# Vill-Lab/2023-TIFS-ISTVT

Measured on AMD Instinct MI355X. Metric: clips/sec (BxTx3x224x224 fwd+bwd), higher is better.
Workload: dtype bf16; 1 GPU; C2: B=32/GPU T=8 224x224 full ISTVT (Xception stem + 12-layer DSTTr) train step (fwd+bwd+grad all-reduce+SGD), random-init weights; global_batch=32, frames=8, size=224, depth=12, parallelism=dp1, early_allreduce=False, attn_fp8=False, dead_row_elimination=False, final_norm_class_rows_only=False, optimizer=SGD(momentum 0.9) fused, step_graphs=False

## Files before the change

2023-tifs-istvt_amd/_lib.py:

```python
import ctypes
import os
from ctypes import c_float, c_int, c_long, c_void_p

_HERE = os.path.dirname(os.path.abspath(__file__))
LIB_PATH = os.environ.get('ISTVT_LIB') or os.path.join(_HERE, 'libistvt_hip.so')

P, I, L, F = c_void_p, c_int, c_long, c_float

SIGNATURES = {
    'istvt_gemm': [P, L, I, P, L, I, P, L, I, I, I, P, P, L, P, I, I, I, F, P, P, I, I, P],
    'istvt_layernorm_fwd': [P, L, P, P, P, L, P, P, L, I, F, I, P],
    'istvt_layernorm_fwd_diff': [P, L, P, P, P, L, P, L, P, P, I, I, I, I, F, I, P],
    'istvt_layernorm_bwd': [P, L, P, L, P, P, P, P, L, P, L, P, P, P, P, L, L, I, I, P],
    'istvt_layernorm_bwd_ws_elems': [L, I],
    'istvt_layernorm_bwd_partial': [P, L, P, L, P, P, P, P, L, P, L, I, P, L, L, I, I, P],
    'istvt_layernorm_bwd_reduce': [P, L, L, I, P, P, P, P],
    'istvt_attn_spatial_fwd': [P, L, P, L, P, I, I, I, I, F, I, P],
    'istvt_attn_spatial_bwd': [P, L, P, P, L, P, P, P, I, I, I, I, F, I, P],
    'istvt_attn_spatial_fwd_fp8': [P, L, P, L, P, I, I, I, I, F, I, P],
    'istvt_attn_spatial_bwd_fp8': [P, L, P, P, L, P, P, P, I, I, I, I, F, I, P],
    'istvt_attn_temporal_fwd': [P, L, P, L, P, L, I, I, I, I, I, F, I, I, P],
    'istvt_attn_temporal_bwd': [P, L, P, L, P, L, P, P, I, I, I, I, I, F, I, I, P],
    'istvt_attn_spatial_relevance': [P, L, P, L, P, P, P, I, I, I, I, F, I, P],
    'istvt_attn_temporal_relevance': [P, L, P, L, P, P, I, I, I, I, I, F, I, I, P],
# ... 17 lines not shown
    'istvt_bn_add_fwd': [P, P, P, P, P, L, I, I, P],
    'istvt_im2col_conv1': [P, P, I, I, I, P],
    'istvt_conv1_fwd': [P, P, P, I, I, I, P],
    'istvt_conv1_fwd_u8': [P, P, P, P, P, I, I, I, P],
    'istvt_conv1_wgrad': [P, P, P, P, I, I, I, P],
    'istvt_conv1_wgrad_slabs': [],
    'istvt_conv1_fwd_u8_view': [P, L, I, I, P, P, P, P, P, I, I, I, P],
    'istvt_conv1_wgrad_u8': [P, P, L, I, I, P, P, P, P, P, I, I, I, P],
    'istvt_im2col_conv1_u8': [P, L, I, I, P, P, P, P, I, I, I, P],
    'istvt_crop_resize_u8': [P, L, I, I, P, P, I, I, P],
    'istvt_jpeg_roundtrip_u8': [P, L, I, I, I, P, I, P, L, P, P],
    'istvt_conv2_fwd': [P, P, P, P, I, I, I, P],
    'istvt_conv2_dgrad': [P, P, P, P, P, I, I, I, P],
    'istvt_conv2_wgrad': [P, P, P, P, P, I, I, I, P],
    'istvt_conv2_wgrad_slabs': [],
    'istvt_col2im_conv1': [P, P, I, I, I, P],
    'istvt_im2col3x3': [P, P, I, P, I, I, I, I, I, P],
    'istvt_col2im3x3': [P, P, P, P, I, I, I, I, I, P],
    'istvt_dwconv3x3': [P, P, P, I, I, I, I, P, I, I, P, P, I, I, P, I, I, P, P, I, P],
    'istvt_dwconv3x3_wgrad': [P, P, I, P, P, P, L, I, I, I, I, I, P],
    'istvt_dwconv3x3_wgrad_ws_elems': [I, I, I, I],
    'istvt_pool_add_fwd': [P, P, P, P, P, P, I, I, I, I, I, P],
    'istvt_pool_bwd': [P, P, P, I, I, I, I, P, P, P, P, I, P],
    'istvt_subsample2': [P, P, I, I, I, I, I, P],
    'istvt_splitk_reduce': [P, I, L, P, P],
    'istvt_wgrad_group': [I, P, P, P, P, P, P, P, I, I, P, L, P],
    'istvt_wgrad_group_splits': [I, P, P, I],
    'istvt_colsum': [P, P, L, I, L, P, L, I, P],
    'istvt_colsum_ws_elems': [L, I],
    'istvt_rows_reduce': [P, I, L, P, P],
# ... 63 lines not shown
```

2023-tifs-istvt_amd/csrc/conv_dense.hip:

```cpp
#include "common.h"
#include "u8_view.h"
#include <type_traits>

namespace {

__device__ __forceinline__ bf16x8 ld_frag(const bf16_t* p) { return *reinterpret_cast<const bf16x8*>(p); }
__device__ __forceinline__ bf16x8 zero_frag() {
    bf16x8 f;
#pragma unroll
    for (int i = 0; i < 8; ++i) f[i] = (bf16_t)0.0f;
    return f;
}
__device__ __forceinline__ f32x4 mma16(const bf16x8& a, const bf16x8& b, const f32x4& c) {
    return __builtin_amdgcn_mfma_f32_16x16x32_bf16(a, b, c, 0, 0, 0);
}

template <typename T>
__device__ __forceinline__ void conv1_mac_store(const float* v, const float* __restrict__ w, T* __restrict__ out) {
#pragma unroll
    for (int c8 = 0; c8 < 4; ++c8) {
        float o[8];
#pragma unroll
        for (int j = 0; j < 8; ++j) {
            const float* wc = w + (c8 * 8 + j) * 27;
            float a = 0.f;
#pragma unroll
            for (int k = 0; k < 27; ++k) a = fmaf(wc[k], v[k], a);
            o[j] = a;
        }
        store8(out + c8 * 8, o);
    }
}

template <typename T>
__global__ __launch_bounds__(256) void conv1_fwd_kernel(const float* __restrict__ x, const float* __restrict__ w,
                                                        T* __restrict__ u1, long Mo, int S, int Ho, int Wo) {
    const long m = (long)blockIdx.x * 256 + threadIdx.x;
    if (m >= Mo) return;
    const int xo = (int)(m % Wo), yo = (int)((m / Wo) % Ho);
    const long f = m / ((long)Wo * Ho);
    float v[27];
#pragma unroll
    for (int ci = 0; ci < 3; ++ci)
#pragma unroll
        for (int dy = 0; dy < 3; ++dy) {
            const float* row = x + ((f * 3 + ci) * S + 2 * yo + dy) * S + 2 * xo;
#pragma unroll
            for (int dx = 0; dx < 3; ++dx) v[ci * 9 + dy * 3 + dx] = row[dx];
        }
    conv1_mac_store(v, w, u1 + m * 32);
}

struct Conv1Mac {
    static __device__ __forceinline__ int slot(int dy, int dx, int ci) { return ci * 9 + dy * 3 + dx; }
    template <typename T>
    static __device__ __forceinline__ void emit(const float* v, const float* __restrict__ w, T* __restrict__ out) {
        int w0 = 0;
        asm volatile("" : "+s"(w0));
        conv1_mac_store(v, w + w0, out);
    }
};

struct Conv1Col {
    static __device__ __forceinline__ int slot(int dy, int dx, int ci) { return (dy * 3 + dx) * 3 + ci; }
    template <typename T>
// ... 34 lines not shown
#pragma unroll
        for (int dy = 0; dy < 3; ++dy) {
            const int rr = 2 * yl + dy;
            const unsigned char* row = sb + rr * pitch + u8_row_lead(lead0, rr, rstride);
#pragma unroll
            for (int dx = 0; dx < 3; ++dx) {
                const unsigned char* px = row + u8_view_px(2 * xo + dx, S, vw.flip);
#pragma unroll
                for (int ci = 0; ci < 3; ++ci) v[Sink::slot(dy, dx, ci)] = lut[ci * 256 + px[ci]];
            }
        }
        Sink::emit(v, w, out + ((f * Ho + yb) * (long)Ho + o) * 32);
    }
}

__global__ __launch_bounds__(256, 2) void conv2_fwd_kernel(const bf16_t* __restrict__ u1, const float* __restrict__ bnp,
                                                           const bf16_t* __restrict__ w, bf16_t* __restrict__ u2, long Mo,
                                                           int H, int W, int Ho, int Wo, int ngroups) {
    const int tid = threadIdx.x, lane = tid & 63, wave = tid >> 6;
    const int r = lane & 15, g = lane >> 4;
    __shared__ bf16x8 wl3[9 * 64];
    bf16x8 wf[9][3];
#pragma unroll
    for (int tap = 0; tap < 9; ++tap) {
#pragma unroll
        for (int nt = 0; nt < 3; ++nt)
            wf[tap][nt] = ld_frag(w + (16 * (r >> 2) + 4 * nt + (r & 3)) * 288 + tap * 32 + 8 * g);
        if (wave == 0) wl3[tap * 64 + lane] = ld_frag(w + (16 * (r >> 2) + 4 * 3 + (r & 3)) * 288 + tap * 32 + 8 * g);
    }
    __syncthreads();
    float mu[8], sc[8], be[8];
    load8(bnp + 8 * g, mu);
    load8(bnp + 2 * 32 + 8 * g, sc);
    load8(bnp + 3 * 32 + 8 * g, be);
    constexpr int RSEG = 9;
    const int nstrips = (Wo + 15) / 16, nsegs = (Ho + RSEG - 1) / RSEG;
// ... 37 lines not shown
                        const bf16x8& xf = ring[(k + dy) % 3][dx];
#pragma unroll
                        for (int nt = 0; nt < 3; ++nt) acc[nt] = mma16(wf[dy * 3 + dx][nt], xf, acc[nt]);
                        acc[3] = mma16(wl3[(dy * 3 + dx) * 64 + lo], xf, acc[3]);
                    }
                if (ok) {
                    bf16x8 o0, o1;
#pragma unroll
                    for (int i = 0; i < 4; ++i) {
                        o0[i] = (bf16_t)acc[0][i]; o0[4 + i] = (bf16_t)acc[1][i];
                        o1[i] = (bf16_t)acc[2][i]; o1[4 + i] = (bf16_t)acc[3][i];
                    }
                    bf16_t* dst = u2 + (((f * Ho + yo) * Wo) + xo) * 64 + 16 * g;
                    *reinterpret_cast<bf16x8*>(dst) = o0;
                    *reinterpret_cast<bf16x8*>(dst + 8) = o1;
                }
            }
        }
    }
}

__global__ __launch_bounds__(256, 2) void conv2_dgrad_kernel(const bf16_t* __restrict__ du2, const bf16_t* __restrict__ w,
                                                             const bf16_t* __restrict__ u1, const float* __restrict__ bnp,
                                                             bf16_t* __restrict__ dz1, long Mi, int H, int W, int Ho,
                                                             int Wo, int ngroups) {
    __shared__ bf16_t wt[9 * 32 * 64];
    const int tid = threadIdx.x, lane = tid & 63, wave = tid >> 6;
    const int r = lane & 15, g = lane >> 4;
    for (int i = tid; i < 64 * 36; i += 256) {
        const int co = i / 36, k8 = (i % 36) * 8;
        const bf16x8 v = ld_frag(w + co * 288 + k8);
#pragma unroll
        for (int j = 0; j < 8; ++j) wt[(k8 + j) * 64 + co] = v[j];
    }
    __syncthreads();
    bf16x8 wf[9][2][2];
#pragma unroll
    for (int tap = 3; tap < 9; ++tap)
#pragma unroll
        for (int ks = 0; ks < 2; ++ks)
#pragma unroll
            for (int nt = 0; nt < 2; ++nt)
                wf[tap][ks][nt] = ld_frag(wt + (tap * 32 + 8 * (r >> 2) + 4 * nt + (r & 3)) * 64 + 32 * ks + 8 * g);
// ... 49 lines not shown
#pragma unroll
                    for (int nt = 0; nt < 2; ++nt)
                        acc[nt] = mma16(ld_frag(wt + (dx * 32 + wo + 4 * nt) * 64 + 32 * ks + wcol), ring[k % 3][dx][ks], acc[nt]);
            if (ok) {
                float mu[8], sc[8], be[8];
                load8(bnp + 8 * g, mu);
                load8(bnp + 2 * 32 + 8 * g, sc);
                load8(bnp + 3 * 32 + 8 * g, be);
                bf16x8 o;
#pragma unroll
                for (int j = 0; j < 8; ++j) {
                    const float z = ((float)uraw[j] - mu[j]) * sc[j] + be[j];
                    o[j] = (bf16_t)(z > 0.f ? acc[j >> 2][j & 3] : 0.f);
                }
                *reinterpret_cast<bf16x8*>(dz1 + m * 32 + 8 * g) = o;
            }
            }
        }
    }
}

constexpr int WG_PX = 32;
constexpr int DIMG_PITCH = 64 * 2 + 16;
constexpr int AIMG_PITCH = 32 * 2 + 16;
constexpr int AIMG_ROWS = WG_PX + 2;

__device__ __forceinline__ bf16x8 tr_frag(const char* img, int pitch, int k0, int col16, int r) {
    typedef short4v __attribute__((address_space(3))) * lds_ptr;
    typedef short short8v __attribute__((ext_vector_type(8)));
    const int q = r >> 2, pp = r & 3;
    const char* pa = img + (k0 + q) * pitch + (col16 + 4 * pp) * 2;
    const char* pb = pa + 4 * pitch;
// ... 239 lines not shown
    const int cap = 256 * per_cu;
    return need < cap ? (need > 0 ? need : 1) : cap;
}

}

extern "C" int istvt_conv1_fwd(const float* x, const float* w, void* u1, int Fr, int S, int dtype, hipStream_t stream) {
    if (Fr <= 0 || S < 3) return ISTVT_ERR_SHAPE;
    const int Ho = (S - 3) / 2 + 1;
    const long Mo = (long)Fr * Ho * Ho;
    DISPATCH_DTYPE(dtype, hipLaunchKernelGGL((conv1_fwd_kernel<T>), dim3((unsigned)((Mo + 255) / 256)), dim3(256), 0,
                                             stream, x, w, (T*)u1, Mo, S, Ho, Ho));
    return istvt_check_launch();
}

static inline bool u8_view_args_ok(const void* x, long total, int Hs, int Ws, const float* mean, const float* stdv, int Fr,
                                   int S) {
    if (Fr <= 0 || S < 3 || !x || !mean || !stdv) return false;
    if (Hs < S || Ws < S || Hs > 16384 || Ws > 16384) return false;
    return total >= (long)Fr * Hs * Ws * 3;
}

template <typename Sink>
static int conv1_u8_launch(const void* x, long total, int Hs, int Ws, const int* view, const float* mean, const float* stdv,
                           const float* w, void* out, int Fr, int S, int dtype, hipStream_t stream) {
    if (!u8_view_args_ok(x, total, Hs, Ws, mean, stdv, Fr, S) || S > 4096 || !out) return ISTVT_ERR_SHAPE;
    const int Ho = (S - 3) / 2 + 1;
    const int pitch = u8_row_pitch(S);
    int R = 1;
    double best = 0.0;
// ... 16 lines not shown
                                       hipStream_t stream) {
    if (!w) return ISTVT_ERR_SHAPE;
    return conv1_u8_launch<Conv1Mac>(x, total, Hs, Ws, view, mean, stdv, w, u1, Fr, S, dtype, stream);
}

extern "C" int istvt_conv1_fwd_u8(const void* x, const float* mean, const float* stdv, const float* w, void* u1, int Fr,
                                  int S, int dtype, hipStream_t stream) {
    return istvt_conv1_fwd_u8_view(x, (long)Fr * S * S * 3, S, S, nullptr, mean, stdv, w, u1, Fr, S, dtype, stream);
}

extern "C" int istvt_im2col_conv1_u8(const void* x, long total, int Hs, int Ws, const int* view, const float* mean,
                                     const float* stdv, void* col, int Fr, int S, int dtype, hipStream_t stream) {
    return conv1_u8_launch<Conv1Col>(x, total, Hs, Ws, view, mean, stdv, nullptr, col, Fr, S, dtype, stream);
}

extern "C" int istvt_conv2_fwd(const void* u1, const float* bnp, const void* w, void* u2, int Fr, int H, int W,
                               hipStream_t stream) {
    if (Fr <= 0 || H < 3 || W < 3 || !bnp) return ISTVT_ERR_SHAPE;
    const int Ho = H - 2, Wo = W - 2;
    const long Mo = (long)Fr * Ho * Wo;
    if (Mo / 16 + 1 > 0x7fffffffL) return ISTVT_ERR_SHAPE;
    const int ngroups = (int)((Mo + 15) / 16);
    const long items = (long)Fr * ((Wo + 15) / 16) * ((Ho + 8) / 9);
    hipLaunchKernelGGL(conv2_fwd_kernel, dim3(wave_grid((int)(items < 0x7fffffffL ? items : 0x7fffffffL), 2)), dim3(256), 0, stream, (const bf16_t*)u1, bnp,
                       (const bf16_t*)w, (bf16_t*)u2, Mo, H, W, Ho, Wo, ngroups);
    return istvt_check_launch();
}

extern "C" int istvt_conv2_dgrad(const void* du2, const void* w, const void* u1, const float* bnp, void* dz1, int Fr,
                                 int H, int W, hipStream_t stream) {
    if (Fr <= 0 || H < 3 || W < 3 || !bnp) return ISTVT_ERR_SHAPE;
    const long Mi = (long)Fr * H * W;
    if (Mi / 16 + 1 > 0x7fffffffL) return ISTVT_ERR_SHAPE;
    const int ngroups = (int)((Mi + 15) / 16);
    const long items = (long)Fr * ((W + 15) / 16) * ((H + 8) / 9);
    hipLaunchKernelGGL(conv2_dgrad_kernel, dim3(wave_grid((int)(items < 0x7fffffffL ? items : 0x7fffffffL), 2)), dim3(256), 0, stream, (const bf16_t*)du2,
                       (const bf16_t*)w, (const bf16_t*)u1, bnp, (bf16_t*)dz1, Mi, H, W, H - 2, W - 2, ngroups);
    return istvt_check_launch();
}

extern "C" int istvt_conv2_wgrad_slabs() { return 768; }

extern "C" int istvt_conv2_wgrad(const void* du2, const void* u1, const float* bnp, float* slabs, float* dw, int Fr,
                                 int H, int W, hipStream_t stream) {
    if (Fr <= 0 || H < 3 || W < 3 || !bnp || !slabs) return ISTVT_ERR_SHAPE;
    const int Ho = H - 2, Wo = W - 2;
    const long nch = (long)Fr * Ho * ((Wo + WG_PX - 1) / WG_PX);
    if (nch > 0x7fffffffL) return ISTVT_ERR_SHAPE;
    const int cap = istvt_conv2_wgrad_slabs();
    const int grid = nch < cap ? (int)nch : cap;
    hipLaunchKernelGGL(conv2_wgrad_kernel, dim3(grid), dim3(256), 0, stream, (const bf16_t*)du2, (const bf16_t*)u1, bnp,
                       slabs, Fr, H, W, Ho, Wo, (int)nch);
    int rc = istvt_check_launch();
// ... 42 lines not shown
```

2023-tifs-istvt_amd/ops.py:

```python
from __future__ import annotations

import os
from typing import Optional

import torch

from . import _lib
from ._common import (G256_MIN, ROW_ALIGN, Tensor, _DT, _c, _ptr, _req, _stream, cast, dtype_code,
                      empty_rows, pad_ld, rows, zeros_rows)
from .weights import (_refresh_derived, _refresh_plain_copies, _static_holders, _transposed_operand,
                      _versions, derived, invalidate_weight_cache, refresh_stale_operands, set_static_addresses,
                      static_addresses, weight_as, weight_cat_as)


gemm_profile = None
kernel_profile = None


class prof:

    def __init__(self, name, nbytes=0, flops=0):
        self.rec = (name, nbytes, flops) if kernel_profile is not None else None

    def __enter__(self):
# ... 712 lines not shown
    return _c(weight.detach())


def _conv1_du1(what: str, du1: Tensor, Fr: int, S: int, device) -> Tensor:
    Ho = (S - 3) // 2 + 1
    if du1.device != device or du1.dim() != 2 or tuple(du1.shape) != (Fr * Ho * Ho, 32):
        raise RuntimeError('%s: du1 must be (%d, 32) on %s, got %s' % (what, Fr * Ho * Ho, device, tuple(du1.shape)))
    return _c(du1)


def _conv1_wgrad_ws(device):
    return (torch.zeros((32, 32), dtype=torch.float32, device=device),
            torch.empty((_lib.lib().istvt_conv1_wgrad_slabs(), 1024), dtype=torch.float32, device=device))


def conv1_fwd(x: Tensor, weight: Tensor, dtype: torch.dtype) -> Tensor:
    x, Fr, S = _float_clip('conv1_fwd', x)
    w = _conv1_w('conv1_fwd', weight, x.device)
    u1 = _conv1_out(Fr, S, dtype, x.device)
    _lib.check(_lib.lib().istvt_conv1_fwd(x.data_ptr(), w.data_ptr(), u1.data_ptr(), Fr, S, _DT[dtype], _stream()),
               'istvt_conv1_fwd')
    return u1


def conv1_wgrad(du1: Tensor, x: Tensor) -> Tensor:
    x, Fr, S = _float_clip('conv1_wgrad', x)
    du1 = _conv1_du1('conv1_wgrad', du1, Fr, S, x.device)
    dW, slabs = _conv1_wgrad_ws(x.device)
    _lib.check(_lib.lib().istvt_conv1_wgrad(du1.data_ptr(), x.data_ptr(), slabs.data_ptr(), dW.data_ptr(), Fr, S,
                                            dtype_code(du1), _stream()), 'istvt_conv1_wgrad')
    return dW


def im2col_conv1(x: Tensor, dtype: torch.dtype) -> Tensor:
# ... 270 lines not shown
```

2023-tifs-istvt_amd/stem.py:

```python
from __future__ import annotations

from typing import List, Optional

import os

import torch
from torch.autograd import Function
from torch.autograd.function import once_differentiable

from . import _lib, ops
from .ops import _c, _ptr, _req, _stream, dtype_code

Tensor = torch.Tensor
BN_EPS = 1e-5
BN_MOMENTUM = 0.1


def out_side(side: int) -> int:
    s = (side - 3) // 2 + 1 - 2
    for _ in range(3):
        s = (s - 1) // 2 + 1
    return s


# ... 186 lines not shown
                raise RuntimeError('the stem\'s byte entry expects channels-last (frames, Hs, Ws, 3) uint8 input, got %s %s'
                                   % (x.dtype, tuple(x.shape)))
            S = x.shape[1] if S is None else S
            if view is None and (x.shape[1] != S or x.shape[2] != S):
                raise RuntimeError('stem expects channels-last (frames, S, S, 3) uint8 input, got %s' % (tuple(x.shape),))
        else:
            if x.dtype == torch.uint8:
                raise RuntimeError('uint8 frames need mean and std (Xception.low_level_features_nhwc(x, dtype, mean, std))')
            if x.dtype != torch.float32:
                raise TypeError('stem input must be float32, got %s' % x.dtype)
            if x.dim() != 4 or x.shape[1] != 3 or x.shape[2] != x.shape[3]:
                raise RuntimeError('stem expects (frames, 3, S, S) input, got %s' % (tuple(x.shape),))
            S = x.shape[2]
        self.x, self.mean, self.std, self.view, self.S, self.inference = _c(x), mean, std, view, S, inference

    def forward(self, weight, dtype):
        if self.mean is None:
            return ops.conv1_fwd(self.x, weight, dtype)
        if self.inference:
            return ops.conv1_fwd_u8(self.x, self.mean, self.std, weight, dtype)
        return ops.conv1_fwd_u8_view(self.x, self.view, self.S, self.mean, self.std, weight, dtype, checked=True)

    def im2col(self, dtype):
        if self.mean is None:
            return ops.im2col_conv1(self.x, dtype)
        return ops.im2col_conv1_u8(self.x, self.view, self.S, self.mean, self.std, dtype, checked=True)

    def wgrad(self, du1):
        if self.mean is None:
            return ops.conv1_wgrad(du1, self.x)
        return ops.conv1_wgrad_u8(du1, self.x, self.view, self.S, self.mean, self.std, checked=True)


class StemFn(Function):

    @staticmethod
    def forward(ctx, x, dtype, training, buffers, src, *params):
        if src.inference and training:
            raise RuntimeError('the stem\'s inference entry needs eval mode: it has no backward')
        Fr, S = src.x.shape[0], src.S
        L = _lib.lib()
        dev = x.device
        P = dict(zip(param_names(), params))
        bufs = {n: (buffers[2 * i], buffers[2 * i + 1]) for i, n in enumerate(bn_names())}
        sv = {}

        def bn(name, u, M, C):
            rm, rv = bufs[name]
            return bn_forward_stats(u, M, C, P[name + '.weight'], P[name + '.bias'], rm, rv, training)

        def pw_bn(name, xin, w, M, C):
            rm, rv = bufs[name]
            return pointwise_bn(xin, w, M, C, P[name + '.weight'], P[name + '.bias'], rm, rv, training)

        H1 = (S - 3) // 2 + 1
        M1 = Fr * H1 * H1
        w1 = _conv1_weight(P['conv1.weight'], dtype)
        if dtype == torch.bfloat16 or src.inference:
            u1 = src.forward(P['conv1.weight'], dtype)
        else:
            u1 = ops.linear_fwd(src.im2col(dtype), w1, blocked=False)
        bn1 = bn('bn1', u1, M1, 32)
        H2 = H1 - 2
        M2 = Fr * H2 * H2
        w2 = _conv2_weight(P['conv2.weight'], dtype)
        if dtype == torch.bfloat16:
            u2 = torch.empty((M2, 64), dtype=dtype, device=dev)
            _lib.check(L.istvt_conv2_fwd(u1.data_ptr(), bn1.ptr(), w2.data_ptr(), u2.data_ptr(), Fr, H1, H1, _stream()),
                       'istvt_conv2_fwd')
        else:
            col2 = torch.empty((M2, 288), dtype=dtype, device=dev)
            _lib.check(L.istvt_im2col3x3(u1.data_ptr(), bn1.ptr(), 1, col2.data_ptr(), Fr, H1, H1, 32, ops._DT[dtype], _stream()),
                       'istvt_im2col3x3')
            u2 = ops.linear_fwd(col2, w2, blocked=False)
            del col2
        bn2 = bn('bn2', u2, M2, 64)
        sv.update(src=src, S=S, Fr=Fr, H1=H1, H2=H2, u1=u1, bn1=bn1, u2=u2, bn2=bn2, w1=w1, w2=w2)

        fuse_in = os.environ.get('ISTVT_STEM_MATERIALISE_A2', '0') != '1'
        X, H = (u2 if fuse_in else bn_apply(u2, bn2, M2, 64, True)), H2
        blocks = []
        for name, cin_, cout, pre_relu in BLOCKS:
            i0 = 1 if pre_relu else 0
            M = Fr * H * H
            Hs = (H - 1) // 2 + 1
            Ms = Fr * Hs * Hs
            wdwA = tap_major(P['%s.rep.%d.conv1.weight' % (name, i0)])
            wpwA = ops.weight_as(P['%s.rep.%d.pointwise.weight' % (name, i0)], dtype, pad=True)
            wdwB = tap_major(P['%s.rep.%d.conv1.weight' % (name, i0 + 3)])
            wpwB = ops.weight_as(P['%s.rep.%d.pointwise.weight' % (name, i0 + 3)], dtype, pad=True)
            wsk = ops.weight_as(P[name + '.skip.weight'], dtype, pad=True)
# ... 111 lines not shown
            del duA
            fused_in = not blk['pre_relu'] and blk['X'] is sv['u2']
            dw_wgrad(sA + '.conv1.weight', blk['X'], dd1, H, cin, sv['bn2'] if fused_in else None, True if fused_in else blk['pre_relu'])
            if blk['pre_relu']:
                dOut = dwconv(dd1, blk['wdwA'], Fr, H, H, cin, flip=True, msrc=blk['X'], mask_pre=True, addsrc=dxs)
            else:
                stats2 = new_stats(cin, dev)
                dOut = dwconv(dd1, blk['wdwA'], Fr, H, H, cin, flip=True, msrc=sv['u2'], m_bn=sv['bn2'], mask_post=True,
                              addsrc=dxs, stats=stats2)
            del dd1
        H1, H2, S = sv['H1'], sv['H2'], sv['S']
        M1, M2 = Fr * H1 * H1, Fr * H2 * H2
        du2 = bn_bwd(dOut, sv['u2'], sv['bn2'], 'bn2', M2, 64, stats=stats2)
        dz1 = torch.empty((M1, 32), dtype=dtype, device=du2.device)
        dW2 = None
        if dtype == torch.bfloat16:
            du2 = du2.contiguous()
            q2 = P['conv2.weight']

            def conv2_wgrad(du=du2, u1=sv['u1'], bn1=sv['bn1']):
                dW = torch.zeros((64, 288), dtype=torch.float32, device=du.device)
                slabs = torch.empty((L.istvt_conv2_wgrad_slabs(), 64 * 288), dtype=torch.float32, device=du.device)
                _lib.check(L.istvt_conv2_wgrad(du.data_ptr(), u1.data_ptr(), bn1.ptr(), slabs.data_ptr(), dW.data_ptr(),
                                               Fr, H1, H1, _stream()), 'istvt_conv2_wgrad')
                return dW.view(64, 3, 3, 32).permute(0, 3, 1, 2)
            if side_on and getattr(q2, '_istvt_fused_grad', False) and q2.grad is not None:
                from . import functional as Fn
                Fn.side_launch(du2.device, lambda: q2.grad.add_(conv2_wgrad()), keep=(du2, sv['u1'], sv['bn1']))
                grads['conv2.weight'] = None
            else:
                dW2 = conv2_wgrad().contiguous()
            _lib.check(L.istvt_conv2_dgrad(du2.data_ptr(), sv['w2'].data_ptr(), sv['u1'].data_ptr(), sv['bn1'].ptr(),
                                           dz1.data_ptr(), Fr, H1, H1, _stream()), 'istvt_conv2_dgrad')
            del du2
        else:
            col2 = torch.empty((M2, 288), dtype=dtype, device=du2.device)
            _lib.check(L.istvt_im2col3x3(sv['u1'].data_ptr(), sv['bn1'].ptr(), 1, col2.data_ptr(), Fr, H1, H1, 32, dtc, _stream()),
                       'istvt_im2col3x3')
            dW2 = ops.linear_wgrad(du2, col2)
            dcol2 = ops.linear_dgrad(du2, sv['w2'], blocked=False)
            del du2, col2
            _lib.check(L.istvt_col2im3x3(dcol2.data_ptr(), sv['u1'].data_ptr(), sv['bn1'].ptr(), dz1.data_ptr(), Fr, H1, H1, 32,
                                         dtc, _stream()),
                       'istvt_col2im3x3')
            del dcol2
        if 'conv2.weight' not in grads:
            grads['conv2.weight'] = dW2 if dtype == torch.bfloat16 else dW2.view(64, 3, 3, 32).permute(0, 3, 1, 2).contiguous()
        du1 = bn_bwd(dz1, sv['u1'], sv['bn1'], 'bn1', M1, 32)
        del dz1
        src = sv['src']
        if dtype == torch.bfloat16 and H1 <= 128:
            dW1 = src.wgrad(du1.contiguous())
            grads['conv1.weight'] = dW1[:, :27].reshape(32, 3, 3, 3).contiguous()
        else:
            dW1 = ops.linear_wgrad(du1, src.im2col(dtype))
            grads['conv1.weight'] = dW1[:, :27].reshape(32, 3, 3, 3).permute(0, 3, 1, 2).contiguous()
        dx = None
        if ctx.need_dx:
            dcol1 = ops.linear_dgrad(du1, sv['w1'], blocked=False)
            dx = torch.empty_like(src.x)
            _lib.check(L.istvt_col2im_conv1(dcol1.data_ptr(), dx.data_ptr(), Fr, S, dtc, _stream()), 'istvt_col2im_conv1')
        ctx.sv = None
        for n in ('conv1.weight', 'conv2.weight'):
# ... 77 lines not shown
```

include/istvt_hip.h:

```cpp
#ifndef ISTVT_HIP_H
#define ISTVT_HIP_H

#ifdef __cplusplus
extern "C" {
#endif

typedef void* istvt_stream_t;

#define ISTVT_F32 0
#define ISTVT_BF16 1

int istvt_gemm(const void* A, long lda, int a_kc, const void* B, long ldb, int b_kc, void* C, long ldc, int M, int N,
               int K, const float* bias, const void* residual, long ldr, void* C2, int epi, int out_mode, int splitk,
               float alpha, double* col_sum, double* col_sumsq, int flags, int dtype, istvt_stream_t stream);

int istvt_splitk_reduce(const float* ws, int splits, long n, float* out, istvt_stream_t stream);

int istvt_wgrad_group(int count, const void* const* dy, const long* lddy, const void* const* x, const long* ldx,
                      float* const* out, const int* N, const int* K, int M, int splits, float* ws, long ws_elems,
                      istvt_stream_t stream);
int istvt_wgrad_group_splits(int count, const int* N, const int* K, int M);

int istvt_layernorm_fwd(const void* x, long ldx, const float* gamma, const float* beta, void* y, long ldy, float* mean,
                        float* rstd, long M, int D, float eps, int dtype, istvt_stream_t stream);
// ... 91 lines not shown
int istvt_conv1_wgrad_u8(const void* du1, const void* x, long total, int Hs, int Ws, const int* view, const float* mean,
                         const float* std, float* slabs, float* dw, int frames, int S, int dtype, istvt_stream_t stream);
int istvt_im2col_conv1_u8(const void* x, long total, int Hs, int Ws, const int* view, const float* mean, const float* std,
                          void* col, int frames, int S, int dtype, istvt_stream_t stream);
int istvt_crop_resize_u8(const void* frames, long total, int Hs, int Ws, const int* boxes, void* out, int n, int S,
                         istvt_stream_t stream);
int istvt_jpeg_roundtrip_u8(const void* frames, long total, int n, int H, int W, const int* quality, int subsampling,
                            void* scratch, long scratch_bytes, void* out, istvt_stream_t stream);
int istvt_conv2_fwd(const void* u1, const float* bnp, const void* w, void* u2, int frames, int H, int W,
                    istvt_stream_t stream);
int istvt_conv2_dgrad(const void* du2, const void* w, const void* u1, const float* bnp, void* dz1, int frames, int H,
                      int W, istvt_stream_t stream);
int istvt_conv2_wgrad(const void* du2, const void* u1, const float* bnp, float* slabs, float* dw, int frames, int H,
                      int W, istvt_stream_t stream);
int istvt_conv2_wgrad_slabs(void);

int istvt_dwconv3x3(const void* in, const float* w, void* out, int frames, int H, int W, int C, const float* in_bn,
                    int in_relu, int flip, const void* msrc, const float* m_bn, int mask_pre, int mask_post,
                    const void* addsrc, int Ha, int Wa, double* st_s1, double* st_s2, int dtype,
                    istvt_stream_t stream);
int istvt_dwconv3x3_wgrad(const void* in, const float* in_bn, int in_relu, const void* dout, float* dw, float* ws,
                          long ws_elems, int frames, int H, int W, int C, int dtype, istvt_stream_t stream);
int istvt_dwconv3x3_wgrad_ws_elems(int frames, int H, int W, int C);

int istvt_pool_add_fwd(const void* x, const float* bnx, const void* skip, const float* bns, void* out,
                       unsigned char* argmax, int frames, int H, int W, int C, int dtype, istvt_stream_t stream);
int istvt_pool_bwd(const void* dout, const unsigned char* argmax, void* dz, int frames, int H, int W, int C,
                   const void* u, const float* bnp, double* s1, double* s2, int dtype, istvt_stream_t stream);
int istvt_subsample2(const void* in, void* out, int frames, int H, int W, int C, int dtype, istvt_stream_t stream);

// ... 74 lines not shown
```

Measured before the change: 634.2 clips/s.

## Fuse BatchNorm statistics into conv1/conv2 forward and conv2 dgrad kernels

Adds stats-fused variants of the stem conv1 forward, conv2 forward and conv2 dgrad kernels. They accumulate per-channel sum and sum-of-squares, or the backward BN reductions, in shared memory and atomically add them into replicated double accumulators. The Python stem passes these accumulators to bn_forward_stats and bn_bwd, so the separate BN stats passes that re-read the large stem activations are skipped. In exchange the kernels gain extra LDS traffic from per-element shared atomics, a larger shared footprint that may lower occupancy, and a different reduction order. An environment variable can switch back to the unfused path.

```diff
diff --git a/2023-tifs-istvt_amd/_lib.py b/2023-tifs-istvt_amd/_lib.py
--- a/2023-tifs-istvt_amd/_lib.py
+++ b/2023-tifs-istvt_amd/_lib.py
@@ -55,6 +55,9 @@
     'istvt_conv2_dgrad': [P, P, P, P, P, I, I, I, P],
     'istvt_conv2_wgrad': [P, P, P, P, P, I, I, I, P],
     'istvt_conv2_wgrad_slabs': [],
+    'istvt_conv1_fwd_stats': [P, P, P, P, P, I, I, I, P],
+    'istvt_conv2_fwd_stats': [P, P, P, P, P, P, I, I, I, P],
+    'istvt_conv2_dgrad_stats': [P, P, P, P, P, P, P, I, I, I, P],
     'istvt_col2im_conv1': [P, P, I, I, I, P],
     'istvt_im2col3x3': [P, P, I, P, I, I, I, I, I, P],
     'istvt_col2im3x3': [P, P, P, P, I, I, I, I, I, P],
diff --git a/2023-tifs-istvt_amd/csrc/conv_dense.hip b/2023-tifs-istvt_amd/csrc/conv_dense.hip
--- a/2023-tifs-istvt_amd/csrc/conv_dense.hip
+++ b/2023-tifs-istvt_amd/csrc/conv_dense.hip
@@ -1,5 +1,6 @@
 #include "common.h"
 #include "u8_view.h"
+#include <cstdlib>
 #include <type_traits>
 
 namespace {
@@ -15,8 +16,8 @@
     return __builtin_amdgcn_mfma_f32_16x16x32_bf16(a, b, c, 0, 0, 0);
 }
 
-template <typename T>
-__device__ __forceinline__ void conv1_mac_store(const float* v, const float* __restrict__ w, T* __restrict__ out) {
+template <typename T, typename Also>
+__device__ __forceinline__ void conv1_mac_store(const float* v, const float* __restrict__ w, T* __restrict__ out, Also also) {
 #pragma unroll
     for (int c8 = 0; c8 < 4; ++c8) {
         float o[8];
@@ -29,7 +30,25 @@
             o[j] = a;
         }
         store8(out + c8 * 8, o);
-    }
+        also(c8, o);
+    }
+}
+template <typename T>
+__device__ __forceinline__ void conv1_mac_store(const float* v, const float* __restrict__ w, T* __restrict__ out) {
+    conv1_mac_store(v, w, out, [](int, const float (&)[8]) {});
+}
+
+__device__ __forceinline__ void conv1_gather(const float* __restrict__ x, long m, int S, int Ho, int Wo, float (&v)[27]) {
+    const int xo = (int)(m % Wo), yo = (int)((m / Wo) % Ho);
+    const long f = m / ((long)Wo * Ho);
+#pragma unroll
+    for (int ci = 0; ci < 3; ++ci)
+#pragma unroll
+        for (int dy = 0; dy < 3; ++dy) {
+            const float* row = x + ((f * 3 + ci) * S + 2 * yo + dy) * S + 2 * xo;
+#pragma unroll
+            for (int dx = 0; dx < 3; ++dx) v[ci * 9 + dy * 3 + dx] = row[dx];
+        }
 }
 
 template <typename T>
@@ -37,18 +56,54 @@
                                                         T* __restrict__ u1, long Mo, int S, int Ho, int Wo) {
     const long m = (long)blockIdx.x * 256 + threadIdx.x;
     if (m >= Mo) return;
-    const int xo = (int)(m % Wo), yo = (int)((m / Wo) % Ho);
-    const long f = m / ((long)Wo * Ho);
     float v[27];
-#pragma unroll
-    for (int ci = 0; ci < 3; ++ci)
-#pragma unroll
-        for (int dy = 0; dy < 3; ++dy) {
-            const float* row = x + ((f * 3 + ci) * S + 2 * yo + dy) * S + 2 * xo;
-#pragma unroll
-            for (int dx = 0; dx < 3; ++dx) v[ci * 9 + dy * 3 + dx] = row[dx];
-        }
+    conv1_gather(x, m, S, Ho, Wo, v);
     conv1_mac_store(v, w, u1 + m * 32);
+}
+
+constexpr int C1S_PITCH = 40;
+template <typename T>
+__global__ __launch_bounds__(256) void conv1_fwd_stats_kernel(const float* __restrict__ x, const float* __restrict__ w,
+                                                              T* __restrict__ u1, double* __restrict__ st_sum,
+                                                              double* __restrict__ st_sumsq, long Mo, int S, int Ho, int Wo,
+                                                              long nbatches) {
+    __shared__ __attribute__((aligned(16))) T simg[256 * C1S_PITCH];
+    __shared__ float sred[2][8][32];
+    const int tid = threadIdx.x;
+    const int sc = tid & 31, sl = tid >> 5;
+    float s1 = 0.f, s2 = 0.f;
+    for (long b = blockIdx.x; b < nbatches; b += gridDim.x) {
+        const long m = b * 256 + tid;
+        T* mine = simg + tid * C1S_PITCH;
+        if (m < Mo) {
+            float v[27];
+            conv1_gather(x, m, S, Ho, Wo, v);
+            conv1_mac_store(v, w, u1 + m * 32, [&](int c8, const float (&o)[8]) { store8(mine + c8 * 8, o); });
+        } else {
+            const float z[8] = {0.f, 0.f, 0.f, 0.f, 0.f, 0.f, 0.f, 0.f};
+#pragma unroll
+            for (int c8 = 0; c8 < 4; ++c8) store8(mine + c8 * 8, z);
+        }
+        __syncthreads();
+#pragma unroll 8
+        for (int i = 0; i < 32; ++i) {
+            const float d = to_f32(simg[(sl * 32 + i) * C1S_PITCH + sc]);
+            s1 += d;
+            s2 = fmaf(d, d, s2);
+        }
+        __syncthreads();
+    }
+    sred[0][sl][sc] = s1;
+    sred[1][sl][sc] = s2;
+    __syncthreads();
+    if (tid < 64) {
+        const int a = tid >> 5;
+        float t = 0.f;
+#pragma unroll
+        for (int k = 0; k < 8; ++k) t += sred[a][k][sc];
+        const long rep = (long)(blockIdx.x % ISTVT_STAT_REPLICAS) * 2 * 32;
+        atomicAdd((a ? st_sumsq : st_sum) + rep + sc, (double)t);
+    }
 }
 
 struct Conv1Mac {
@@ -113,12 +168,24 @@
     }
 }
 
+
+__device__ __forceinline__ void lds_add(float* slot, float v) {
+    __hip_atomic_fetch_add(slot, v, __ATOMIC_RELAXED, __HIP_MEMORY_SCOPE_WORKGROUP);
+}
+
+template <bool STATS>
 __global__ __launch_bounds__(256, 2) void conv2_fwd_kernel(const bf16_t* __restrict__ u1, const float* __restrict__ bnp,
-                                                           const bf16_t* __restrict__ w, bf16_t* __restrict__ u2, long Mo,
-                                                           int H, int W, int Ho, int Wo, int ngroups) {
+                                                           const bf16_t* __restrict__ w, bf16_t* __restrict__ u2,
+                                                           double* __restrict__ st_sum, double* __restrict__ st_sumsq,
+                                                           long Mo, int H, int W, int Ho, int Wo, int ngroups) {
     const int tid = threadIdx.x, lane = tid & 63, wave = tid >> 6;
     const int r = lane & 15, g = lane >> 4;
     __shared__ bf16x8 wl3[9 * 64];
+    __shared__ float sacc[STATS ? 32 * 256 : 1];
+    if constexpr (STATS) {
+#pragma unroll
+        for (int e = 0; e < 32; ++e) sacc[e * 256 + tid] = 0.f;
+    }
     bf16x8 wf[9][3];
 #pragma unroll
     for (int tap = 0; tap < 9; ++tap) {
@@ -186,19 +253,49 @@
                     bf16_t* dst = u2 + (((f * Ho + yo) * Wo) + xo) * 64 + 16 * g;
                     *reinterpret_cast<bf16x8*>(dst) = o0;
                     *reinterpret_cast<bf16x8*>(dst + 8) = o1;
+                    if constexpr (STATS) {
+#pragma unroll
+                        for (int e = 0; e < 8; ++e) {
+                            const float d0 = (float)o0[e], d1 = (float)o1[e];
+                            lds_add(sacc + e * 256 + tid, d0);
+                            lds_add(sacc + (16 + e) * 256 + tid, d0 * d0);
+                            lds_add(sacc + (8 + e) * 256 + tid, d1);
+                            lds_add(sacc + (24 + e) * 256 + tid, d1 * d1);
+                        }
+                    }
                 }
             }
         }
     }
-}
-
+    if constexpr (STATS) {
+        __syncthreads();
+        if (tid < 128) {
+            const int a = tid >> 6, c = tid & 63;
+            const float* slots = sacc + (a * 16 + (c & 15)) * 256 + (c >> 4) * 16;
+            float t = 0.f;
+            for (int wv = 0; wv < 4; ++wv)
+#pragma unroll
+                for (int k = 0; k < 16; ++k) t += slots[wv * 64 + k];
+            const long rep = (long)(blockIdx.x % ISTVT_STAT_REPLICAS) * 2 * 64;
+            atomicAdd((a ? st_sumsq : st_sum) + rep + c, (double)t);
+        }
+    }
+}
+
+template <bool STATS>
 __global__ __launch_bounds__(256, 2) void conv2_dgrad_kernel(const bf16_t* __restrict__ du2, const bf16_t* __restrict__ w,
                                                              const bf16_t* __restrict__ u1, const float* __restrict__ bnp,
-                                                             bf16_t* __restrict__ dz1, long Mi, int H, int W, int Ho,
+                                                             bf16_t* __restrict__ dz1, double* __restrict__ st_s1,
+                                                             double* __restrict__ st_s2, long Mi, int H, int W, int Ho,
                                                              int Wo, int ngroups) {
     __shared__ bf16_t wt[9 * 32 * 64];
+    __shared__ float sacc[STATS ? 16 * 256 : 1];
     const int tid = threadIdx.x, lane = tid & 63, wave = tid >> 6;
     const int r = lane & 15, g = lane >> 4;
+    if constexpr (STATS) {
+#pragma unroll
+        for (int j = 0; j < 16; ++j) sacc[j * 256 + tid] = 0.f;
+    }
     for (int i = tid; i < 64 * 36; i += 256) {
         const int co = i / 36, k8 = (i % 36) * 8;
         const bf16x8 v = ld_frag(w + co * 288 + k8);
@@ -278,8 +375,31 @@
                     o[j] = (bf16_t)(z > 0.f ? acc[j >> 2][j & 3] : 0.f);
                 }
                 *reinterpret_cast<bf16x8*>(dz1 + m * 32 + 8 * g) = o;
+                if constexpr (STATS) {
+                    float rs[8];
+                    load8(bnp + 32 + 8 * g, rs);
+#pragma unroll
+                    for (int j = 0; j < 8; ++j) {
+                        const float d = (float)o[j];
+                        lds_add(sacc + j * 256 + tid, d);
+                        lds_add(sacc + (8 + j) * 256 + tid, d * ((float)uraw[j] - mu[j]) * rs[j]);
+                    }
+                }
             }
             }
+        }
+    }
+    if constexpr (STATS) {
+        __syncthreads();
+        if (tid < 64) {
+            const int a = tid >> 5, c = tid & 31;
+            const float* slots = sacc + (a * 8 + (c & 7)) * 256 + (c >> 3) * 16;
+            float t = 0.f;
+            for (int wv = 0; wv < 4; ++wv)
+#pragma unroll
+                for (int k = 0; k < 16; ++k) t += slots[wv * 64 + k];
+            const long rep = (long)(blockIdx.x % ISTVT_STAT_REPLICAS) * 2 * 32;
+            atomicAdd((a ? st_s2 : st_s1) + rep + c, (double)t);
         }
     }
 }
@@ -549,6 +669,30 @@
     return istvt_check_launch();
 }
 
+extern "C" int istvt_bn_stats(const void* x, double* sum, double* sumsq, long M, int C, int dtype, hipStream_t stream);
+extern "C" int istvt_bn_bwd_stats(const void* dz, const void* u, const float* bnp, double* s1, double* s2, long M, int C,
+                                  int dtype, hipStream_t stream);
+static bool conv_stats_fused() {
+    static const bool on = [] { const char* v = getenv("ISTVT_CONV_STATS_FUSED"); return !(v && atoi(v) == 0); }();
+    return on;
+}
+
+extern "C" int istvt_conv1_fwd_stats(const float* x, const float* w, void* u1, double* sum, double* sumsq, int Fr, int S,
+                                     int dtype, hipStream_t stream) {
+    if (Fr <= 0 || S < 3 || !sum || !sumsq) return ISTVT_ERR_SHAPE;
+    const int Ho = (S - 3) / 2 + 1;
+    const long Mo = (long)Fr * Ho * Ho;
+    if (!conv_stats_fused()) {
+        const int rc = istvt_conv1_fwd(x, w, u1, Fr, S, dtype, stream);
+        return rc != ISTVT_OK ? rc : istvt_bn_stats(u1, sum, sumsq, Mo, 32, dtype, stream);
+    }
+    const long nb = (Mo + 255) / 256;
+    const int grid = (int)(nb < 4096 ? nb : 4096);
+    DISPATCH_DTYPE(dtype, hipLaunchKernelGGL((conv1_fwd_stats_kernel<T>), dim3(grid), dim3(256), 0, stream, x, w, (T*)u1,
+                                             sum, sumsq, Mo, S, Ho, Ho, nb));
+    return istvt_check_launch();
+}
+
 static inline bool u8_view_args_ok(const void* x, long total, int Hs, int Ws, const float* mean, const float* stdv, int Fr,
                                    int S) {
     if (Fr <= 0 || S < 3 || !x || !mean || !stdv) return false;
@@ -595,29 +739,65 @@
     return conv1_u8_launch<Conv1Col>(x, total, Hs, Ws, view, mean, stdv, nullptr, col, Fr, S, dtype, stream);
 }
 
-extern "C" int istvt_conv2_fwd(const void* u1, const float* bnp, const void* w, void* u2, int Fr, int H, int W,
-                               hipStream_t stream) {
+static int conv2_fwd_launch(const void* u1, const float* bnp, const void* w, void* u2, double* sum, double* sumsq, int Fr,
+                            int H, int W, hipStream_t stream) {
     if (Fr <= 0 || H < 3 || W < 3 || !bnp) return ISTVT_ERR_SHAPE;
     const int Ho = H - 2, Wo = W - 2;
     const long Mo = (long)Fr * Ho * Wo;
     if (Mo / 16 + 1 > 0x7fffffffL) return ISTVT_ERR_SHAPE;
     const int ngroups = (int)((Mo + 15) / 16);
     const long items = (long)Fr * ((Wo + 15) / 16) * ((Ho + 8) / 9);
-    hipLaunchKernelGGL(conv2_fwd_kernel, dim3(wave_grid((int)(items < 0x7fffffffL ? items : 0x7fffffffL), 2)), dim3(256), 0, stream, (const bf16_t*)u1, bnp,
-                       (const bf16_t*)w, (bf16_t*)u2, Mo, H, W, Ho, Wo, ngroups);
+    const dim3 grid(wave_grid((int)(items < 0x7fffffffL ? items : 0x7fffffffL), 2));
+    if (sum)
+        hipLaunchKernelGGL(conv2_fwd_kernel<true>, grid, dim3(256), 0, stream, (const bf16_t*)u1, bnp, (const bf16_t*)w,
+                           (bf16_t*)u2, sum, sumsq, Mo, H, W, Ho, Wo, ngroups);
+    else
+        hipLaunchKernelGGL(conv2_fwd_kernel<false>, grid, dim3(256), 0, stream, (const bf16_t*)u1, bnp, (const bf16_t*)w,
+                           (bf16_t*)u2, nullptr, nullptr, Mo, H, W, Ho, Wo, ngroups);
     return istvt_check_launch();
 }
 
-extern "C" int istvt_conv2_dgrad(const void* du2, const void* w, const void* u1, const float* bnp, void* dz1, int Fr,
-                                 int H, int W, hipStream_t stream) {
+extern "C" int istvt_conv2_fwd(const void* u1, const float* bnp, const void* w, void* u2, int Fr, int H, int W,
+                               hipStream_t stream) {
+    return conv2_fwd_launch(u1, bnp, w, u2, nullptr, nullptr, Fr, H, W, stream);
+}
+
+extern "C" int istvt_conv2_fwd_stats(const void* u1, const float* bnp, const void* w, void* u2, double* sum, double* sumsq,
+                                     int Fr, int H, int W, hipStream_t stream) {
+    if (!sum || !sumsq) return ISTVT_ERR_SHAPE;
+    if (conv_stats_fused()) return conv2_fwd_launch(u1, bnp, w, u2, sum, sumsq, Fr, H, W, stream);
+    const int rc = conv2_fwd_launch(u1, bnp, w, u2, nullptr, nullptr, Fr, H, W, stream);
+    return rc != ISTVT_OK ? rc : istvt_bn_stats(u2, sum, sumsq, (long)Fr * (H - 2) * (W - 2), 64, DT_BF16, stream);
+}
+
+static int conv2_dgrad_launch(const void* du2, const void* w, const void* u1, const float* bnp, void* dz1, double* s1,
+                              double* s2, int Fr, int H, int W, hipStream_t stream) {
     if (Fr <= 0 || H < 3 || W < 3 || !bnp) return ISTVT_ERR_SHAPE;
     const long Mi = (long)Fr * H * W;
     if (Mi / 16 + 1 > 0x7fffffffL) return ISTVT_ERR_SHAPE;
     const int ngroups = (int)((Mi + 15) / 16);
     const long items = (long)Fr * ((W + 15) / 16) * ((H + 8) / 9);
-    hipLaunchKernelGGL(conv2_dgrad_kernel, dim3(wave_grid((int)(items < 0x7fffffffL ? items : 0x7fffffffL), 2)), dim3(256), 0, stream, (const bf16_t*)du2,
-                       (const bf16_t*)w, (const bf16_t*)u1, bnp, (bf16_t*)dz1, Mi, H, W, H - 2, W - 2, ngroups);
+    const dim3 grid(wave_grid((int)(items < 0x7fffffffL ? items : 0x7fffffffL), 2));
+    if (s1)
+        hipLaunchKernelGGL(conv2_dgrad_kernel<true>, grid, dim3(256), 0, stream, (const bf16_t*)du2, (const bf16_t*)w,
+                           (const bf16_t*)u1, bnp, (bf16_t*)dz1, s1, s2, Mi, H, W, H - 2, W - 2, ngroups);
+    else
+        hipLaunchKernelGGL(conv2_dgrad_kernel<false>, grid, dim3(256), 0, stream, (const bf16_t*)du2, (const bf16_t*)w,
+                           (const bf16_t*)u1, bnp, (bf16_t*)dz1, nullptr, nullptr, Mi, H, W, H - 2, W - 2, ngroups);
     return istvt_check_launch();
+}
+
+extern "C" int istvt_conv2_dgrad(const void* du2, const void* w, const void* u1, const float* bnp, void* dz1, int Fr,
+                                 int H, int W, hipStream_t stream) {
+    return conv2_dgrad_launch(du2, w, u1, bnp, dz1, nullptr, nullptr, Fr, H, W, stream);
+}
+
+extern "C" int istvt_conv2_dgrad_stats(const void* du2, const void* w, const void* u1, const float* bnp, void* dz1,
+                                       double* s1, double* s2, int Fr, int H, int W, hipStream_t stream) {
+    if (!s1 || !s2) return ISTVT_ERR_SHAPE;
+    if (conv_stats_fused()) return conv2_dgrad_launch(du2, w, u1, bnp, dz1, s1, s2, Fr, H, W, stream);
+    const int rc = conv2_dgrad_launch(du2, w, u1, bnp, dz1, nullptr, nullptr, Fr, H, W, stream);
+    return rc != ISTVT_OK ? rc : istvt_bn_bwd_stats(dz1, u1, bnp, s1, s2, (long)Fr * H * W, 32, DT_BF16, stream);
 }
 
 extern "C" int istvt_conv2_wgrad_slabs() { return 768; }
diff --git a/2023-tifs-istvt_amd/ops.py b/2023-tifs-istvt_amd/ops.py
--- a/2023-tifs-istvt_amd/ops.py
+++ b/2023-tifs-istvt_amd/ops.py
@@ -750,10 +750,15 @@
             torch.empty((_lib.lib().istvt_conv1_wgrad_slabs(), 1024), dtype=torch.float32, device=device))
 
 
-def conv1_fwd(x: Tensor, weight: Tensor, dtype: torch.dtype) -> Tensor:
+def conv1_fwd(x: Tensor, weight: Tensor, dtype: torch.dtype, stats: Optional[Tensor] = None) -> Tensor:
     x, Fr, S = _float_clip('conv1_fwd', x)
     w = _conv1_w('conv1_fwd', weight, x.device)
     u1 = _conv1_out(Fr, S, dtype, x.device)
+    if stats is not None:
+        _lib.check(_lib.lib().istvt_conv1_fwd_stats(x.data_ptr(), w.data_ptr(), u1.data_ptr(), stats[0, 0].data_ptr(),
+                                                    stats[0, 1].data_ptr(), Fr, S, _DT[dtype], _stream()),
+                   'istvt_conv1_fwd_stats')
+        return u1
     _lib.check(_lib.lib().istvt_conv1_fwd(x.data_ptr(), w.data_ptr(), u1.data_ptr(), Fr, S, _DT[dtype], _stream()),
                'istvt_conv1_fwd')
     return u1
diff --git a/2023-tifs-istvt_amd/stem.py b/2023-tifs-istvt_amd/stem.py
--- a/2023-tifs-istvt_amd/stem.py
+++ b/2023-tifs-istvt_amd/stem.py
@@ -224,9 +224,13 @@
             S = x.shape[2]
         self.x, self.mean, self.std, self.view, self.S, self.inference = _c(x), mean, std, view, S, inference
 
-    def forward(self, weight, dtype):
+    def takes_stats(self) -> bool:
+        return self.mean is None
+
+    def forward(self, weight, dtype, stats=None):
         if self.mean is None:
-            return ops.conv1_fwd(self.x, weight, dtype)
+            return ops.conv1_fwd(self.x, weight, dtype, stats=stats)
+        assert stats is None
         if self.inference:
             return ops.conv1_fwd_u8(self.x, self.mean, self.std, weight, dtype)
         return ops.conv1_fwd_u8_view(self.x, self.view, self.S, self.mean, self.std, weight, dtype, checked=True)
@@ -255,9 +259,9 @@
         bufs = {n: (buffers[2 * i], buffers[2 * i + 1]) for i, n in enumerate(bn_names())}
         sv = {}
 
-        def bn(name, u, M, C):
+        def bn(name, u, M, C, acc=None):
             rm, rv = bufs[name]
-            return bn_forward_stats(u, M, C, P[name + '.weight'], P[name + '.bias'], rm, rv, training)
+            return bn_forward_stats(u, M, C, P[name + '.weight'], P[name + '.bias'], rm, rv, training, acc=acc)
 
         def pw_bn(name, xin, w, M, C):
             rm, rv = bufs[name]
@@ -266,25 +270,35 @@
         H1 = (S - 3) // 2 + 1
         M1 = Fr * H1 * H1
         w1 = _conv1_weight(P['conv1.weight'], dtype)
+        acc1 = None
         if dtype == torch.bfloat16 or src.inference:
-            u1 = src.forward(P['conv1.weight'], dtype)
+            if training and src.takes_stats():
+                acc1 = new_stats(32, dev)
+            u1 = src.forward(P['conv1.weight'], dtype, stats=acc1)
         else:
             u1 = ops.linear_fwd(src.im2col(dtype), w1, blocked=False)
-        bn1 = bn('bn1', u1, M1, 32)
+        bn1 = bn('bn1', u1, M1, 32, acc1)
         H2 = H1 - 2
         M2 = Fr * H2 * H2
         w2 = _conv2_weight(P['conv2.weight'], dtype)
+        acc2 = None
         if dtype == torch.bfloat16:
             u2 = torch.empty((M2, 64), dtype=dtype, device=dev)
-            _lib.check(L.istvt_conv2_fwd(u1.data_ptr(), bn1.ptr(), w2.data_ptr(), u2.data_ptr(), Fr, H1, H1, _stream()),
-                       'istvt_conv2_fwd')
+            if training:
+                acc2 = new_stats(64, dev)
+                _lib.check(L.istvt_conv2_fwd_stats(u1.data_ptr(), bn1.ptr(), w2.data_ptr(), u2.data_ptr(),
+                                                   acc2[0, 0].data_ptr(), acc2[0, 1].data_ptr(), Fr, H1, H1, _stream()),
+                           'istvt_conv2_fwd_stats')
+            else:
+                _lib.check(L.istvt_conv2_fwd(u1.data_ptr(), bn1.ptr(), w2.data_ptr(), u2.data_ptr(), Fr, H1, H1, _stream()),
+                           'istvt_conv2_fwd')
         else:
             col2 = torch.empty((M2, 288), dtype=dtype, device=dev)
             _lib.check(L.istvt_im2col3x3(u1.data_ptr(), bn1.ptr(), 1, col2.data_ptr(), Fr, H1, H1, 32, ops._DT[dtype], _stream()),
                        'istvt_im2col3x3')
             u2 = ops.linear_fwd(col2, w2, blocked=False)
             del col2
-        bn2 = bn('bn2', u2, M2, 64)
+        bn2 = bn('bn2', u2, M2, 64, acc2)
         sv.update(src=src, S=S, Fr=Fr, H1=H1, H2=H2, u1=u1, bn1=bn1, u2=u2, bn2=bn2, w1=w1, w2=w2)
 
         fuse_in = os.environ.get('ISTVT_STEM_MATERIALISE_A2', '0') != '1'
@@ -426,6 +440,7 @@
         du2 = bn_bwd(dOut, sv['u2'], sv['bn2'], 'bn2', M2, 64, stats=stats2)
         dz1 = torch.empty((M1, 32), dtype=dtype, device=du2.device)
         dW2 = None
+        stats1 = None
         if dtype == torch.bfloat16:
             du2 = du2.contiguous()
             q2 = P['conv2.weight']
@@ -442,8 +457,14 @@
                 grads['conv2.weight'] = None
             else:
                 dW2 = conv2_wgrad().contiguous()
-            _lib.check(L.istvt_conv2_dgrad(du2.data_ptr(), sv['w2'].data_ptr(), sv['u1'].data_ptr(), sv['bn1'].ptr(),
-                                           dz1.data_ptr(), Fr, H1, H1, _stream()), 'istvt_conv2_dgrad')
+            if training:
+                stats1 = new_stats(32, du2.device)
+                _lib.check(L.istvt_conv2_dgrad_stats(du2.data_ptr(), sv['w2'].data_ptr(), sv['u1'].data_ptr(), sv['bn1'].ptr(),
+                                                     dz1.data_ptr(), stats1[0, 0].data_ptr(), stats1[0, 1].data_ptr(),
+                                                     Fr, H1, H1, _stream()), 'istvt_conv2_dgrad_stats')
+            else:
+                _lib.check(L.istvt_conv2_dgrad(du2.data_ptr(), sv['w2'].data_ptr(), sv['u1'].data_ptr(), sv['bn1'].ptr(),
+                                               dz1.data_ptr(), Fr, H1, H1, _stream()), 'istvt_conv2_dgrad')
             del du2
         else:
             col2 = torch.empty((M2, 288), dtype=dtype, device=du2.device)
@@ -458,7 +479,7 @@
             del dcol2
         if 'conv2.weight' not in grads:
             grads['conv2.weight'] = dW2 if dtype == torch.bfloat16 else dW2.view(64, 3, 3, 32).permute(0, 3, 1, 2).contiguous()
-        du1 = bn_bwd(dz1, sv['u1'], sv['bn1'], 'bn1', M1, 32)
+        du1 = bn_bwd(dz1, sv['u1'], sv['bn1'], 'bn1', M1, 32, stats=stats1)
         del dz1
         src = sv['src']
         if dtype == torch.bfloat16 and H1 <= 128:
diff --git a/include/istvt_hip.h b/include/istvt_hip.h
--- a/include/istvt_hip.h
+++ b/include/istvt_hip.h
@@ -129,6 +129,12 @@
 int istvt_conv2_wgrad(const void* du2, const void* u1, const float* bnp, float* slabs, float* dw, int frames, int H,
                       int W, istvt_stream_t stream);
 int istvt_conv2_wgrad_slabs(void);
+int istvt_conv1_fwd_stats(const float* x, const float* w, void* u1, double* sum, double* sumsq, int frames, int S,
+                          int dtype, istvt_stream_t stream);
+int istvt_conv2_fwd_stats(const void* u1, const float* bnp, const void* w, void* u2, double* sum, double* sumsq,
+                          int frames, int H, int W, istvt_stream_t stream);
+int istvt_conv2_dgrad_stats(const void* du2, const void* w, const void* u1, const float* bnp, void* dz1, double* s1,
+                            double* s2, int frames, int H, int W, istvt_stream_t stream);
 
 int istvt_dwconv3x3(const void* in, const float* w, void* out, int frames, int H, int W, int C, const float* in_bn,
                     int in_relu, int flip, const void* msrc, const float* m_bn, int mask_pre, int mask_post,
```

Measured after the change: 600.1 clips/s. 0.946x the previous value.
